# OpenDriveLab/kai0

Measured on AMD Instinct MI355X. Metric: train samples/sec pi0.5 full FT, higher is better.
Workload: dtype bf16; 1 GPU; pi0.5 full fine-tune bf16, batch 32 per MI355X, 3-cam 224x224 (BASELINE.json configs[1]); global_batch=32, seq_len=1018, parallelism=dp1

## Files before the change

kai0_amd/csrc/gemm_bf16.hip:

```cpp
#include "common.h"
#include "../../include/kai0hip.h"
#include <stdlib.h>
#include <algorithm>
#include <atomic>
#include <type_traits>

namespace {

constexpr int BK = 64;

#ifdef KAI0_ABLATE
#define KAI0_ABL(p) ((p).ablate)
#else
#define KAI0_ABL(p) 0
#endif

struct RowMap {
    int32_t rpb;
    int64_t bs, off;
    __device__ __forceinline__ int64_t operator()(int r) const {
        if (rpb == 0) return r;
        const int q = r / rpb;
        return (int64_t)q * bs + (r - q * rpb) + off;
    }
// ... 161 lines not shown
        }
        *reinterpret_cast<f32x4*>(cp) = f32x4{v[0], v[1], v[2], v[3]};
        *reinterpret_cast<f32x4*>(cp + 4) = f32x4{v[4], v[5], v[6], v[7]};
    } else {
        bf16_t* cp = reinterpret_cast<bf16_t*>(cbase) + cz + orow * p.ldc + ccol;
        if (p.nseg > 0) {
            int si = 0;
            if (p.nseg > 1 && ccol >= p.seg_begin[1]) si = 1;
            if (p.nseg > 2 && ccol >= p.seg_begin[2]) si = 2;
            cp = p.seg_dst[si] + orow * p.seg_ld[si] + (ccol - p.seg_begin[si]);
        }
        if (p.accumulate) {
            bf16x8 ov = *reinterpret_cast<const bf16x8*>(cp);
#pragma unroll
            for (int e = 0; e < 8; ++e) v[e] += bf2f(ov[e]);
        }
        bf16x8 ov;
#pragma unroll
        for (int e = 0; e < 8; ++e) ov[e] = f2bf(v[e]);
        store_pre8(cp, ov, p.nt_c);
    }
}

#define N_ALIGNED8(n) (((n) & 7) == 0)

__device__ __forceinline__ void lds_barrier() {
    __builtin_amdgcn_sched_barrier(0);
    asm volatile("s_waitcnt lgkmcnt(0)" ::: "memory");
    __builtin_amdgcn_s_barrier();
    asm volatile("" ::: "memory");
    __builtin_amdgcn_sched_barrier(0);
}

template <bool A_KC, bool B_KC, int WM, int WN, int MT, int NT, bool PP, int NS = 2, int BKT = 64, int SCH = 0>
__global__ __launch_bounds__(WM * WN * 64, (WM * WN * 64) / 256) void gemm_bf16_kernel(const GemmArgs p) {
    static_assert(PP ? (WM == 2 && WN == 4 && MT == 8 && ((SCH == 1 && NS == 2 && BKT == 64) || (SCH == 3 && NS == 4 && BKT == 32)))
                     : (SCH == 0 && NS >= 2 && BKT == 64),
                  "K loops: plain multi-stage (SCH 0, 64 deep), quadrant (SCH 1: 256x256x64, 2 stages), ring (SCH 3: 256x256x32, 4 slots)");
    constexpr int BK = BKT;
    constexpr int NWAVES = WM * WN;
    constexpr int TBM = WM * MT * 16, TBN = WN * NT * 16;
    constexpr int A_TILE = TBM * BK * 2, B_TILE = TBN * BK * 2;
    constexpr int STAGE = A_TILE + B_TILE;
    constexpr int NA = A_TILE / 1024 / NWAVES;
    constexpr int NB = B_TILE / 1024 / NWAVES;
    constexpr int KC_CPR = BK / 8;
// ... 371 lines not shown
    #pragma unroll
                    for (int t = 0; t < AH; ++t) af[t] = load_frag(ta, A_KC, A_ROWB, wm * (MT * 16) + (h * AH + t) * 16, ks);
    #pragma unroll
                    for (int i = 0; i < AH; ++i)
    #pragma unroll
                        for (int j = 0; j < NT; ++j)
                            acc[h * AH + i][j] = __builtin_amdgcn_mfma_f32_16x16x32_bf16(af[i], bfr[j], acc[h * AH + i][j], 0, 0, 0);
                }
            }
            slot_c = slot_c + 1 == NS ? 0 : slot_c + 1;
            slot_p = slot_p + 1 == NS ? 0 : slot_p + 1;
        }
        lds_barrier();
    }

    float* slab = reinterpret_cast<float*>(smem + wave * (AH * 4096));
    const int64_t cz = z1 * p.sC1 + z2 * p.sC2;
    const int64_t rz = z1 * p.sR1 + z2 * p.sR2;
    const int64_t vz = z1 * p.rv_s1 + z2 * p.rv_s2;
    constexpr bool ILM = SCH == 1 && !A_KC, ILN = SCH == 1 && !B_KC;
    const int ccol = ILN ? n0 + ((lane & 7) >> 2) * 128 + wn * 32 + ((lane & 7) & 3) * 8 : n0 + wn * 64 + (lane & 7) * 8;
    auto row_base = [&](int h) { return ILM ? m0 + h * 128 + wm * 64 : m0 + wm * (MT * 16) + h * 64; };
    const bool col_ok = ccol < ((p.N + 7) & ~7);
    const bool fused_fast = p.act >= 2 && p.split_k == 1 && p.bias == nullptr && p.gate == nullptr && p.residual == nullptr &&
                            !p.accumulate && !p.out_f32 && p.nseg == 0 && (p.act == 4 || p.scale == 1.0f) &&
                            (p.act != 3 || p.pre_out != nullptr);
    const bool plain_fast = p.act <= 1 && p.split_k == 1 && (p.bias != nullptr || p.residual != nullptr) && p.gate == nullptr &&
                            !p.accumulate && !p.out_f32 && p.nseg == 0 && (N_ALIGNED8(p.N));
    const bool simple_fast = MT == 8 && p.simple_epi && p.act <= 1 && p.split_k == 1 && p.gate == nullptr && !p.out_f32 && p.scale == 1.0f &&
                             p.cmap.rpb == 0 && (N_ALIGNED8(p.N));
    auto epi_half = [&](auto hc) {
        constexpr int h = decltype(hc)::value;
        if constexpr (((MT == 4 && WM == 2) || (MT == 2 && WM == 4)) && WN == 2 && A_KC && B_KC) if (p.act == 7) {
            const bool rot = n0 < p.rope_n_end;
            const int fi = ((n0 >> 7) & 1) * 64 + (lane & 7) * 8;
            const int rcol = rot ? (n0 >> 8) * 256 + wn * 128 + fi : n0 + wn * 64 + (lane & 7) * 8;
            const int rbase = row_base(h) + (lane >> 3);
            bf16x8 cs[AH * 2], sn[AH * 2];
#pragma unroll
            for (int it = 0; it < AH * 2; ++it) {
                const int64_t tr = (int64_t)min(rbase + it * 8, p.M - 1) * p.rope_half + fi;
                cs[it] = *reinterpret_cast<const bf16x8*>(p.rope_cos + (rot ? tr : 0));
                sn[it] = *reinterpret_cast<const bf16x8*>(p.rope_sin + (rot ? tr : 0));
            }
#pragma unroll
            for (int i = 0; i < AH; ++i)
#pragma unroll
                for (int j = 0; j < 4; ++j)
#pragma unroll
                    for (int r = 0; r < 4; ++r) slab[(i * 16 + 4 * g + r) * 64 + j * 16 + l15] = acc[i][j][r];
            lds_barrier();
            const float* pslab = reinterpret_cast<const float*>(smem + (wave ^ 1) * (AH * 4096));
            int si = 0;
// ... 47 lines not shown
                const float gv[8] = {g0[0], g0[1], g0[2], g0[3], g1[0], g1[1], g1[2], g1[3]};
                const float uv[8] = {u0[0], u0[1], u0[2], u0[3], u1[0], u1[1], u1[2], u1[3]};
                bf16x8 gb, ub, hb;
#pragma unroll
                for (int e = 0; e < 8; e += 2) {
                    const f32x2 gr = rbf2(f32x2{gv[e], gv[e + 1]}), ur = rbf2(f32x2{uv[e], uv[e + 1]});
                    const f32x2 hv = rbf2(gelu_tanh2(gr)) * ur;
                    gb[e] = f2bf(gr[0]);
                    gb[e + 1] = f2bf(gr[1]);
                    ub[e] = f2bf(ur[0]);
                    ub[e + 1] = f2bf(ur[1]);
                    hb[e] = f2bf(hv[0]);
                    hb[e + 1] = f2bf(hv[1]);
                }
                const int64_t o = cz + p.cmap(row) * p.ldc + ocol;
                *reinterpret_cast<bf16x8*>(cb + o) = hb;
                if (p.pre_out != nullptr) store_pre8(p.pre_out + o, gb, p.nt_pre);
                if (p.pre_out2 != nullptr) store_pre8(p.pre_out2 + o, ub, p.nt_pre);
            }
            asm volatile("s_waitcnt lgkmcnt(0)" ::: "memory");
            __builtin_amdgcn_wave_barrier();
            return;
        }
        if constexpr (MT != 2) if (fused_fast) {
            bf16x8 s0[8], s1[8];
            float ds[8];
            const int rbase = row_base(h) + (lane >> 3);
#pragma unroll
            for (int it = 0; it < 8; ++it) {
                const int row = rbase + it * 8;
                s0[it] = bf16x8{};
                s1[it] = bf16x8{};
                ds[it] = 0.f;
                if (row < p.M && col_ok) {
                    const int64_t o = cz + p.cmap(row) * p.ldc + ccol;
                    s0[it] = *reinterpret_cast<const bf16x8*>(p.aux1 + o);
                    if (p.act == 3) s1[it] = *reinterpret_cast<const bf16x8*>(p.aux2 + o);
                    if (p.act == 4) ds[it] = p.rowvec[vz + (int64_t)row * p.rv_ld];
                }
            }
#pragma unroll
            for (int i = 0; i < 4; ++i)
#pragma unroll
                for (int j = 0; j < 4; ++j)
#pragma unroll
                    for (int r = 0; r < 4; ++r) slab[(i * 16 + 4 * g + r) * 64 + j * 16 + l15] = acc[h * 4 + i][j][r];
            asm volatile("s_waitcnt lgkmcnt(0)" ::: "memory");
// ... 110 lines not shown
                        store_pre8(p.pre_out + o, pv, p.nt_pre);
                    }
#pragma unroll
                    for (int e = 0; e < 8; e += 2) {
                        const f32x2 a = gelu_tanh2(f32x2{v[e], v[e + 1]});
                        v[e] = rbf(a[0]);
                        v[e + 1] = rbf(a[1]);
                    }
                }
                if (p.residual != nullptr) {
#pragma unroll
                    for (int e = 0; e < 8; ++e) v[e] = rbf(v[e] + bf2f(rs[it][e]));
                }
                bf16x8 ov;
#pragma unroll
                for (int e = 0; e < 8; ++e) ov[e] = f2bf(v[e]);
                *reinterpret_cast<bf16x8*>(cb + o) = ov;
            }
            asm volatile("s_waitcnt lgkmcnt(0)" ::: "memory");
            __builtin_amdgcn_wave_barrier();
            return;
        }
        if constexpr (MT == 8) if (simple_fast) {
            const bool has_bias = p.bias != nullptr, has_res = p.residual != nullptr, gelu = p.act == 1;
            const int M_ = p.M, nt_pre_ = p.nt_pre, nt_c_ = p.nt_c;
            const bf16_t* res_ = p.residual;
            bf16_t* pre_ = p.pre_out;
            const int64_t ldr_ = p.ldr, ldc_ = p.ldc;
            float bv[8] = {0.f, 0.f, 0.f, 0.f, 0.f, 0.f, 0.f, 0.f};
            if (has_bias && col_ok) {
                if (p.bias_f32) {
                    const f32x4 b0 = *reinterpret_cast<const f32x4*>(reinterpret_cast<const float*>(p.bias) + ccol);
                    const f32x4 b1 = *reinterpret_cast<const f32x4*>(reinterpret_cast<const float*>(p.bias) + ccol + 4);
#pragma unroll
                    for (int e = 0; e < 4; ++e) { bv[e] = b0[e]; bv[4 + e] = b1[e]; }
                } else {
                    const bf16x8 b = *reinterpret_cast<const bf16x8*>(reinterpret_cast<const bf16_t*>(p.bias) + ccol);
#pragma unroll
                    for (int e = 0; e < 8; ++e) bv[e] = bf2f(b[e]);
                }
            }
            bf16_t* cl = reinterpret_cast<bf16_t*>(p.C) + cz + ccol;
            int64_t ldl = p.ldc;
            if (p.nseg > 0) {
                cl = p.seg_dst[0] + (ccol - p.seg_begin[0]);
                ldl = p.seg_ld[0];
                if (p.nseg > 1 && ccol >= p.seg_begin[1]) {
                    cl = p.seg_dst[1] + (ccol - p.seg_begin[1]);
                    ldl = p.seg_ld[1];
                }
                if (p.nseg > 2 && ccol >= p.seg_begin[2]) {
                    cl = p.seg_dst[2] + (ccol - p.seg_begin[2]);
                    ldl = p.seg_ld[2];
                }
            }
            const int rbase = row_base(h) + (lane >> 3);
            auto res_row = [&](int it) -> bf16x8 {
                const int row = rbase + it * 8;
                return (has_res && row < M_ && col_ok) ? *reinterpret_cast<const bf16x8*>(res_ + rz + (int64_t)row * ldr_ + ccol) : bf16x8{};
            };
            const bool accum = p.accumulate != 0;
            auto old_row = [&](int it) -> bf16x8 {
                const int row = rbase + it * 8;
                return (accum && row < M_ && col_ok) ? *reinterpret_cast<const bf16x8*>(cl + (int64_t)row * ldl) : bf16x8{};
            };
            bf16x8 rnext = res_row(0), onext = old_row(0);
#pragma unroll
            for (int i = 0; i < 4; ++i)
#pragma unroll
                for (int j = 0; j < 4; ++j)
#pragma unroll
                    for (int r = 0; r < 4; ++r) slab[(i * 16 + 4 * g + r) * 64 + j * 16 + l15] = acc[h * 4 + i][j][r];
            asm volatile("s_waitcnt lgkmcnt(0)" ::: "memory");
            __builtin_amdgcn_wave_barrier();
#pragma unroll
            for (int it = 0; it < 8; ++it) {
                const int row = rbase + it * 8;
                const float* sp = slab + (it * 8 + (lane >> 3)) * 64 + (lane & 7) * 8;
                const f32x4 v0 = *reinterpret_cast<const f32x4*>(sp);
                const f32x4 v1 = *reinterpret_cast<const f32x4*>(sp + 4);
                const bf16x8 rv = rnext, ov0 = onext;
                if (it + 1 < 8) {
                    rnext = res_row(it + 1);
                    onext = old_row(it + 1);
                }
                if (row >= M_ || !col_ok) continue;
                float v[8] = {v0[0], v0[1], v0[2], v0[3], v1[0], v1[1], v1[2], v1[3]};
                if (has_bias) {
#pragma unroll
                    for (int e = 0; e < 8; ++e) v[e] += bv[e];
                }
#pragma unroll
                for (int e = 0; e < 8; ++e) v[e] = rbf(v[e]);
                if (gelu) {
                    if (pre_ != nullptr) {
                        bf16x8 pv;
#pragma unroll
                        for (int e = 0; e < 8; ++e) pv[e] = f2bf(v[e]);
                        store_pre8(pre_ + cz + (int64_t)row * ldc_ + ccol, pv, nt_pre_);
                    }
#pragma unroll
                    for (int e = 0; e < 8; e += 2) {
                        const f32x2 a = gelu_tanh2(f32x2{v[e], v[e + 1]});
                        v[e] = rbf(a[0]);
                        v[e + 1] = rbf(a[1]);
                    }
                }
                if (has_res) {
#pragma unroll
                    for (int e = 0; e < 8; ++e) v[e] = rbf(v[e] + bf2f(rv[e]));
                }
                if (accum) {
#pragma unroll
                    for (int e = 0; e < 8; ++e) v[e] += bf2f(ov0[e]);
                }
                bf16x8 ov;
#pragma unroll
                for (int e = 0; e < 8; ++e) ov[e] = f2bf(v[e]);
                store_pre8(cl + (int64_t)row * ldl, ov, nt_c_);
            }
            asm volatile("s_waitcnt lgkmcnt(0)" ::: "memory");
            __builtin_amdgcn_wave_barrier();
            return;
        }
#pragma unroll
        for (int i = 0; i < AH; ++i)
#pragma unroll
            for (int j = 0; j < 4; ++j)
#pragma unroll
                for (int r = 0; r < 4; ++r) slab[(i * 16 + 4 * g + r) * 64 + j * 16 + l15] = acc[h * AH + i][j][r];
        asm volatile("s_waitcnt lgkmcnt(0)" ::: "memory");
        __builtin_amdgcn_wave_barrier();
#pragma unroll 1
        for (int it = 0; it < AH * 2; ++it) {
            const int lr = it * 8 + (lane >> 3);
            const int row = row_base(h) + lr;
            if (row >= p.M || !col_ok) continue;
            const float* sp = slab + lr * 64 + (lane & 7) * 8;
            f32x4 v0 = *reinterpret_cast<const f32x4*>(sp);
            f32x4 v1 = *reinterpret_cast<const f32x4*>(sp + 4);
            float v[8] = {v0[0], v0[1], v0[2], v0[3], v1[0], v1[1], v1[2], v1[3]};
            if (p.split_k > 1) {
                float* wp = reinterpret_cast<float*>(p.ws) + ((int64_t)blockIdx.y * p.M + row) * p.N + ccol;
                *reinterpret_cast<f32x4*>(wp) = v0;
                *reinterpret_cast<f32x4*>(wp + 4) = v1;
            } else {
                epilogue8(p, v, row, ccol, cz, rz, vz, p.C, p.out_f32 != 0);
            }
        }
        asm volatile("s_waitcnt lgkmcnt(0)" ::: "memory");
        __builtin_amdgcn_wave_barrier();
    };
    epi_half(std::integral_constant<int, 0>{});
    if constexpr (MT / 4 > 1) epi_half(std::integral_constant<int, 1>{});
    if constexpr (MT / 4 > 2) epi_half(std::integral_constant<int, 2>{});
    static_assert(MT / 4 <= 3, "extend the epilogue parts");
}

constexpr int PS_SLOTS = 1024;
__device__ unsigned int g_ps_ctr[PS_SLOTS][16];

#ifdef KAI0_PS_TRACE
__device__ long long g_ps_trace[256][8];
#define PS_STAMP(i)                                              \
    do {                                                         \
        const long long n_ = __builtin_amdgcn_s_memrealtime();   \
        t_acc[i] += n_ - t_prev;                                 \
        t_prev = n_;                                             \
    } while (0)
#else
#define PS_STAMP(i) do { } while (0)
#endif

__global__ __launch_bounds__(512, 1) void gemm_nt_persistent_kernel(const GemmArgs p, unsigned int* __restrict__ ctr) {
    constexpr int TBM = 256, TBN = 256, A_TILE = TBM * BK * 2, STAGE = 2 * A_TILE, GROUP = 4, MT = 8;
    extern __shared__ __attribute__((aligned(16))) char smem[];
    const int tid = threadIdx.x, lane = tid & 63;
    const int wave = __builtin_amdgcn_readfirstlane(tid >> 6);
// ... 159 lines not shown
            read_a(ta, 1);
            __builtin_amdgcn_sched_barrier(0);
            issue_half(false, 0, t + 2);
            lds_barrier();
            quad(I1{}, I1{});
            lds_barrier();
            read_b(tb, 0);
            __builtin_amdgcn_sched_barrier(0);
            issue_half(true, 1, t + 2);
            asm volatile("s_waitcnt vmcnt(6)" ::: "memory");
            lds_barrier();
            quad(I1{}, I0{});
            lds_barrier();
        }
        asm volatile("s_waitcnt vmcnt(0)" ::: "memory");
        if (grp == 0) lds_barrier();
        lds_barrier();

        PS_STAMP(1);
        const int m0c = m0, n0c = n0;
        int nn = -1;
        unsigned raw = 0;
        if (tid == 0 && nxt >= 0) raw = draw();
        if (nxt >= 0) {
            setup(nxt);
            prologue_issue();
        }
        const int ccol = n0c + wn * 64 + (lane & 7) * 8;
        const bool col_ok = ccol < ((p.N + 7) & ~7);
        const bool fused_fast = p.act >= 2 && p.act <= 5 && p.bias == nullptr && p.gate == nullptr && p.residual == nullptr && !p.accumulate &&
                                !p.out_f32 && p.nseg == 0 && (p.act == 4 || p.scale == 1.0f) && (p.act != 3 || p.pre_out != nullptr);
        const bool simple_fast = p.simple_epi && p.act <= 1 && p.split_k == 1 && p.gate == nullptr && !p.out_f32 && p.scale == 1.0f && p.cmap.rpb == 0 &&
                                 (N_ALIGNED8(p.N));
        auto to_slab = [&](int ti) {
            __builtin_amdgcn_wave_barrier();
#pragma unroll
            for (int j = 0; j < 4; ++j)
#pragma unroll
                for (int r = 0; r < 4; ++r) slab[(4 * g + r) * 64 + j * 16 + l15] = acc[ti][j][r];
            asm volatile("s_waitcnt lgkmcnt(0)" ::: "memory");
            __builtin_amdgcn_wave_barrier();
        };
        if (pair) {
            const int ocol = (n0c >> 1) + wn * 32 + (lane & 3) * 8;
            const bool ocol_ok = ocol < (p.N >> 1);
            bf16_t* cb = reinterpret_cast<bf16_t*>(p.C);
#pragma unroll
            for (int ti = 0; ti < MT; ++ti) {
                to_slab(ti);
                const int row = m0c + wm * 128 + ti * 16 + (lane >> 2);
                const float* sp = slab + (lane >> 2) * 64 + (lane & 3) * 8;
                const f32x4 g0 = *reinterpret_cast<const f32x4*>(sp), g1 = *reinterpret_cast<const f32x4*>(sp + 4);
                const f32x4 u0 = *reinterpret_cast<const f32x4*>(sp + 32), u1 = *reinterpret_cast<const f32x4*>(sp + 36);
                if (row < p.M && ocol_ok) {
                    const float gv[8] = {g0[0], g0[1], g0[2], g0[3], g1[0], g1[1], g1[2], g1[3]};
                    const float uv[8] = {u0[0], u0[1], u0[2], u0[3], u1[0], u1[1], u1[2], u1[3]};
                    bf16x8 gb, ub, hb;
#pragma unroll
                    for (int e = 0; e < 8; e += 2) {
                        const f32x2 gr = rbf2(f32x2{gv[e], gv[e + 1]}), ur = rbf2(f32x2{uv[e], uv[e + 1]});
                        const f32x2 hv = rbf2(gelu_tanh2(gr)) * ur;
                        gb[e] = f2bf(gr[0]); gb[e + 1] = f2bf(gr[1]);
                        ub[e] = f2bf(ur[0]); ub[e + 1] = f2bf(ur[1]);
                        hb[e] = f2bf(hv[0]); hb[e + 1] = f2bf(hv[1]);
                    }
                    const int64_t o = p.cmap(row) * p.ldc + ocol;
                    *reinterpret_cast<bf16x8*>(cb + o) = hb;
                    if (p.pre_out != nullptr) store_pre8(p.pre_out + o, gb, p.nt_pre);
                    if (p.pre_out2 != nullptr) store_pre8(p.pre_out2 + o, ub, p.nt_pre);
                }
            }
        } else if (fused_fast) {
            bf16_t* cb = reinterpret_cast<bf16_t*>(p.C);
#pragma unroll
            for (int h = 0; h < 2; ++h) {
                bf16x8 s0[8], s1[8];
                float ds[8];
                const int rbase = m0c + wm * 128 + h * 64 + (lane >> 3);
#pragma unroll
                for (int it = 0; it < 8; ++it) {
                    const int row = rbase + it * 8;
                    s0[it] = bf16x8{};
                    s1[it] = bf16x8{};
                    ds[it] = 0.f;
                    if (row < p.M && col_ok) {
                        const int64_t o = p.cmap(row) * p.ldc + ccol;
                        s0[it] = *reinterpret_cast<const bf16x8*>(p.aux1 + o);
                        if (p.act == 3) s1[it] = *reinterpret_cast<const bf16x8*>(p.aux2 + o);
                        if (p.act == 4) ds[it] = p.rowvec[(int64_t)row * p.rv_ld];
                    }
                }
#pragma unroll
                for (int i = 0; i < 4; ++i) {
                    to_slab(h * 4 + i);
#pragma unroll
                    for (int it2 = 0; it2 < 2; ++it2) {
                        const int it = 2 * i + it2;
                        const int row = rbase + it * 8;
                        const float* sp = slab + (it2 * 8 + (lane >> 3)) * 64 + (lane & 7) * 8;
                        const f32x4 v0 = *reinterpret_cast<const f32x4*>(sp), v1 = *reinterpret_cast<const f32x4*>(sp + 4);
                        const float v[8] = {v0[0], v0[1], v0[2], v0[3], v1[0], v1[1], v1[2], v1[3]};
                        if (row >= p.M || !col_ok) continue;
                        const int64_t o = p.cmap(row) * p.ldc + ccol;
                        bf16x8 ov;
                        if (p.act == 2) {
                            if (p.pre_out != nullptr) {
                                bf16x8 uv;
#pragma unroll
                                for (int e = 0; e < 8; ++e) uv[e] = f2bf(v[e]);
                                *reinterpret_cast<bf16x8*>(p.pre_out + o) = uv;
                            }
#pragma unroll
                            for (int e = 0; e < 8; e += 2) {
                                const f32x2 r = rbf2(gelu_tanh2(f32x2{bf2f(s0[it][e]), bf2f(s0[it][e + 1])})) * rbf2(f32x2{v[e], v[e + 1]});
                                ov[e] = f2bf(r[0]);
                                ov[e + 1] = f2bf(r[1]);
                            }
                        } else if (p.act == 3) {
                            bf16x8 du;
#pragma unroll
                            for (int e = 0; e < 8; e += 2) {
                                const f32x2 dh = rbf2(f32x2{v[e], v[e + 1]});
                                f32x2 gl, gr;
                                gelu_tanh_both2(f32x2{bf2f(s0[it][e]), bf2f(s0[it][e + 1])}, gl, gr);
                                const f32x2 a = dh * rbf2(gl);
                                const f32x2 b = rbf2(dh * f32x2{bf2f(s1[it][e]), bf2f(s1[it][e + 1])}) * gr;
                                du[e] = f2bf(a[0]); du[e + 1] = f2bf(a[1]);
                                ov[e] = f2bf(b[0]); ov[e + 1] = f2bf(b[1]);
                            }
                            *reinterpret_cast<bf16x8*>(p.pre_out + o) = du;
                        } else if (p.act == 5) {
#pragma unroll
                            for (int e = 0; e < 8; e += 2) {
                                f32x2 gl, gr;
                                gelu_tanh_both2(f32x2{bf2f(s0[it][e]), bf2f(s0[it][e + 1])}, gl, gr);
                                const f32x2 b = rbf2(f32x2{v[e], v[e + 1]}) * gr;
                                ov[e] = f2bf(b[0]); ov[e + 1] = f2bf(b[1]);
                            }
                        } else {
#pragma unroll
                            for (int e = 0; e < 8; ++e) ov[e] = f2bf((bf2f(s0[it][e]) * (v[e] - ds[it])) * p.scale);
                        }
                        *reinterpret_cast<bf16x8*>(cb + o) = ov;
                    }
                }
            }
        } else if (simple_fast) {
            const bool has_bias = p.bias != nullptr, has_res = p.residual != nullptr, gelu = p.act == 1;
            const int M_ = p.M, nt_pre_ = p.nt_pre, nt_c_ = p.nt_c;
            const bf16_t* res_ = p.residual;
            bf16_t* pre_ = p.pre_out;
            const int64_t ldr_ = p.ldr, ldc_ = p.ldc;
            float bv[8] = {0.f, 0.f, 0.f, 0.f, 0.f, 0.f, 0.f, 0.f};
            if (has_bias && col_ok) {
                if (p.bias_f32) {
                    const f32x4 b0 = *reinterpret_cast<const f32x4*>(reinterpret_cast<const float*>(p.bias) + ccol);
                    const f32x4 b1 = *reinterpret_cast<const f32x4*>(reinterpret_cast<const float*>(p.bias) + ccol + 4);
#pragma unroll
                    for (int e = 0; e < 4; ++e) { bv[e] = b0[e]; bv[4 + e] = b1[e]; }
                } else {
                    const bf16x8 b = *reinterpret_cast<const bf16x8*>(reinterpret_cast<const bf16_t*>(p.bias) + ccol);
#pragma unroll
                    for (int e = 0; e < 8; ++e) bv[e] = bf2f(b[e]);
                }
            }
            bf16_t* cl = reinterpret_cast<bf16_t*>(p.C) + ccol;
            int64_t ldl = p.ldc;
            if (p.nseg > 0) {
                cl = p.seg_dst[0] + (ccol - p.seg_begin[0]);
                ldl = p.seg_ld[0];
                if (p.nseg > 1 && ccol >= p.seg_begin[1]) {
                    cl = p.seg_dst[1] + (ccol - p.seg_begin[1]);
                    ldl = p.seg_ld[1];
                }
                if (p.nseg > 2 && ccol >= p.seg_begin[2]) {
                    cl = p.seg_dst[2] + (ccol - p.seg_begin[2]);
                    ldl = p.seg_ld[2];
                }
            }
            const int rbase = m0c + wm * 128 + (lane >> 3);
            auto res_row = [&](int k) -> bf16x8 {
                const int row = rbase + k * 8;
                return (has_res && row < M_ && col_ok) ? *reinterpret_cast<const bf16x8*>(res_ + (int64_t)row * ldr_ + ccol) : bf16x8{};
            };
            const bool accum = p.accumulate != 0;
            auto old_row = [&](int k) -> bf16x8 {
                const int row = rbase + k * 8;
                return (accum && row < M_ && col_ok) ? *reinterpret_cast<const bf16x8*>(cl + (int64_t)row * ldl) : bf16x8{};
            };
            bf16x8 rnext = res_row(0), onext = old_row(0);
#pragma unroll
            for (int ti = 0; ti < MT; ++ti) {
                to_slab(ti);
#pragma unroll
                for (int it2 = 0; it2 < 2; ++it2) {
                    const int k = ti * 2 + it2;
                    const int row = rbase + k * 8;
                    const float* sp = slab + (it2 * 8 + (lane >> 3)) * 64 + (lane & 7) * 8;
                    const f32x4 v0 = *reinterpret_cast<const f32x4*>(sp), v1 = *reinterpret_cast<const f32x4*>(sp + 4);
                    const bf16x8 rv = rnext, ov0 = onext;
                    if (k + 1 < 2 * MT) {
                        rnext = res_row(k + 1);
                        onext = old_row(k + 1);
                    }
                    if (row >= M_ || !col_ok) continue;
                    float v[8] = {v0[0], v0[1], v0[2], v0[3], v1[0], v1[1], v1[2], v1[3]};
                    if (has_bias) {
#pragma unroll
                        for (int e = 0; e < 8; ++e) v[e] += bv[e];
                    }
#pragma unroll
                    for (int e = 0; e < 8; ++e) v[e] = rbf(v[e]);
                    if (gelu) {
                        if (pre_ != nullptr) {
                            bf16x8 pv;
#pragma unroll
                            for (int e = 0; e < 8; ++e) pv[e] = f2bf(v[e]);
                            store_pre8(pre_ + (int64_t)row * ldc_ + ccol, pv, nt_pre_);
                        }
#pragma unroll
                        for (int e = 0; e < 8; e += 2) {
                            const f32x2 a = gelu_tanh2(f32x2{v[e], v[e + 1]});
                            v[e] = rbf(a[0]);
                            v[e + 1] = rbf(a[1]);
                        }
                    }
                    if (has_res) {
#pragma unroll
                        for (int e = 0; e < 8; ++e) v[e] = rbf(v[e] + bf2f(rv[e]));
                    }
                    if (accum) {
#pragma unroll
                        for (int e = 0; e < 8; ++e) v[e] += bf2f(ov0[e]);
                    }
                    bf16x8 ov;
#pragma unroll
                    for (int e = 0; e < 8; ++e) ov[e] = f2bf(v[e]);
                    store_pre8(cl + (int64_t)row * ldl, ov, nt_c_);
                }
            }
        } else {
#pragma unroll
            for (int ti = 0; ti < MT; ++ti) {
                to_slab(ti);
#pragma unroll 1
                for (int it2 = 0; it2 < 2; ++it2) {
                    const int lr = it2 * 8 + (lane >> 3);
                    const int row = m0c + wm * 128 + ti * 16 + lr;
                    if (row >= p.M || !col_ok) continue;
                    const float* sp = slab + lr * 64 + (lane & 7) * 8;
                    const f32x4 v0 = *reinterpret_cast<const f32x4*>(sp), v1 = *reinterpret_cast<const f32x4*>(sp + 4);
                    float v[8] = {v0[0], v0[1], v0[2], v0[3], v1[0], v1[1], v1[2], v1[3]};
                    epilogue8(p, v, row, ccol, cz, rz, vz, p.C, p.out_f32 != 0);
                }
            }
        }
        PS_STAMP(2);
        __builtin_amdgcn_wave_barrier();
        if (tid == 0) mbox[0] = nxt >= 0 ? resolve(raw) : -1;
        asm volatile("s_waitcnt vmcnt(0)" ::: "memory");
        lds_barrier();
        nn = mbox[0];
        cur = nxt;
        nxt = nn;
// ... 374 lines not shown
```

Measured before the change: 68.14 samples/s.

## Prefetch GEMM epilogue operands through a multi-row register ring with specialized fast paths

The fused and simple GEMM epilogues now fetch their auxiliary, residual and accumulate operands EPI_AHEAD row steps ahead into a register ring, instead of one row ahead. The first loads are issued before the accumulator-to-LDS slab write so global memory latency overlaps with that work. Interior tiles get compile-time specialized variants (fixed activation, residual-only or accumulate-only) that drop bounds checks and runtime branches. The cost is more live registers in the epilogue, which may raise register pressure or lower occupancy, plus extra template instantiations.

```diff
diff --git a/kai0_amd/csrc/gemm_bf16.hip b/kai0_amd/csrc/gemm_bf16.hip
--- a/kai0_amd/csrc/gemm_bf16.hip
+++ b/kai0_amd/csrc/gemm_bf16.hip
@@ -207,6 +207,63 @@
     }
 }
 
+template <int ACT>
+__device__ __forceinline__ void fused_row8(const int act_rt, const float scale, const float (&v)[8], const bf16x8 a1, const bf16x8 a2,
+                                           const float dsum, const int64_t o, bf16_t* cb, bf16_t* pre) {
+    const int act = ACT ? ACT : act_rt;
+    bf16x8 ov;
+    if (act == 2) {
+        if (pre != nullptr) {
+            bf16x8 uv;
+#pragma unroll
+            for (int e = 0; e < 8; ++e) uv[e] = f2bf(v[e]);
+            *reinterpret_cast<bf16x8*>(pre + o) = uv;
+        }
+#pragma unroll
+        for (int e = 0; e < 8; e += 2) {
+            const f32x2 r = rbf2(gelu_tanh2(f32x2{bf2f(a1[e]), bf2f(a1[e + 1])})) * rbf2(f32x2{v[e], v[e + 1]});
+            ov[e] = f2bf(r[0]);
+            ov[e + 1] = f2bf(r[1]);
+        }
+    } else if (act == 3) {
+        bf16x8 du;
+#pragma unroll
+        for (int e = 0; e < 8; e += 2) {
+            const f32x2 dh = rbf2(f32x2{v[e], v[e + 1]});
+            f32x2 gl, gr;
+            gelu_tanh_both2(f32x2{bf2f(a1[e]), bf2f(a1[e + 1])}, gl, gr);
+            const f32x2 a = dh * rbf2(gl);
+            const f32x2 b = rbf2(dh * f32x2{bf2f(a2[e]), bf2f(a2[e + 1])}) * gr;
+            du[e] = f2bf(a[0]);
+            du[e + 1] = f2bf(a[1]);
+            ov[e] = f2bf(b[0]);
+            ov[e + 1] = f2bf(b[1]);
+        }
+        *reinterpret_cast<bf16x8*>(pre + o) = du;
+    } else if (act == 5) {
+#pragma unroll
+        for (int e = 0; e < 8; e += 2) {
+            f32x2 gl, gr;
+            gelu_tanh_both2(f32x2{bf2f(a1[e]), bf2f(a1[e + 1])}, gl, gr);
+            const f32x2 b = rbf2(f32x2{v[e], v[e + 1]}) * gr;
+            ov[e] = f2bf(b[0]);
+            ov[e + 1] = f2bf(b[1]);
+        }
+    } else {
+#pragma unroll
+        for (int e = 0; e < 8; ++e) ov[e] = f2bf((bf2f(a1[e]) * (v[e] - dsum)) * scale);
+    }
+    *reinterpret_cast<bf16x8*>(cb + o) = ov;
+}
+
+#ifndef KAI0_EPI_AHEAD
+#define KAI0_EPI_AHEAD 4
+#endif
+constexpr int EPI_AHEAD = KAI0_EPI_AHEAD;
+template <int V>
+using IC = std::integral_constant<int, V>;
+static_assert(EPI_AHEAD >= 1 && EPI_AHEAD <= 8, "the ring holds EPI_AHEAD row steps of operands in registers");
+
 #define N_ALIGNED8(n) (((n) & 7) == 0)
 
 __device__ __forceinline__ void lds_barrier() {
@@ -624,13 +681,20 @@
     const int ccol = ILN ? n0 + ((lane & 7) >> 2) * 128 + wn * 32 + ((lane & 7) & 3) * 8 : n0 + wn * 64 + (lane & 7) * 8;
     auto row_base = [&](int h) { return ILM ? m0 + h * 128 + wm * 64 : m0 + wm * (MT * 16) + h * 64; };
     const bool col_ok = ccol < ((p.N + 7) & ~7);
-    const bool fused_fast = p.act >= 2 && p.split_k == 1 && p.bias == nullptr && p.gate == nullptr && p.residual == nullptr &&
+    const bool fused_fast = p.simple_epi && p.act >= 2 && p.split_k == 1 && p.bias == nullptr && p.gate == nullptr && p.residual == nullptr &&
                             !p.accumulate && !p.out_f32 && p.nseg == 0 && (p.act == 4 || p.scale == 1.0f) &&
                             (p.act != 3 || p.pre_out != nullptr);
     const bool plain_fast = p.act <= 1 && p.split_k == 1 && (p.bias != nullptr || p.residual != nullptr) && p.gate == nullptr &&
                             !p.accumulate && !p.out_f32 && p.nseg == 0 && (N_ALIGNED8(p.N));
     const bool simple_fast = MT == 8 && p.simple_epi && p.act <= 1 && p.split_k == 1 && p.gate == nullptr && !p.out_f32 && p.scale == 1.0f &&
                              p.cmap.rpb == 0 && (N_ALIGNED8(p.N));
+    bf16x8 es0[EPI_AHEAD], es1[EPI_AHEAD];
+    float eds[EPI_AHEAD];
+    float ebv[8];
+    bf16_t* ecl;
+    int64_t eldl;
+    auto step_row = [&](int k) { return row_base(k >> 3) + (k & 7) * 8 + (lane >> 3); };
+    const bool inner = m0 + TBM <= p.M && n0 + TBN <= ((p.N + 7) & ~7);
     auto epi_half = [&](auto hc) {
         constexpr int h = decltype(hc)::value;
         if constexpr (((MT == 4 && WM == 2) || (MT == 2 && WM == 4)) && WN == 2 && A_KC && B_KC) if (p.act == 7) {
@@ -724,7 +788,71 @@
             __builtin_amdgcn_wave_barrier();
             return;
         }
-        if constexpr (MT != 2) if (fused_fast) {
+        if constexpr (MT == 8) if (fused_fast) {
+            const int M_ = p.M, act_ = p.act;
+            auto run_fused = [&](auto actc, auto innerc) {
+                constexpr int ACT = decltype(actc)::value;
+                constexpr bool INNER = decltype(innerc)::value;
+                const float scale_ = p.scale;
+                const RowMap cmap_ = p.cmap;
+                const int64_t ldc_ = p.ldc, rv_ld_ = p.rv_ld;
+                const bf16_t* aux1_ = p.aux1;
+                const bf16_t* aux2_ = p.aux2;
+                const float* rowvec_ = p.rowvec;
+                bf16_t* pre_ = p.pre_out;
+                auto fetch_aux = [&](int k) {
+                    const int row = step_row(k), sl = k % EPI_AHEAD;
+                    es0[sl] = bf16x8{};
+                    es1[sl] = bf16x8{};
+                    eds[sl] = 0.f;
+                    if (INNER || (row < M_ && col_ok)) {
+                        const int64_t o = cz + cmap_(row) * ldc_ + ccol;
+                        es0[sl] = *reinterpret_cast<const bf16x8*>(aux1_ + o);
+                        if (ACT == 3 || (ACT == 0 && act_ == 3)) es1[sl] = *reinterpret_cast<const bf16x8*>(aux2_ + o);
+                        if (ACT == 0 && act_ == 4) eds[sl] = rowvec_[vz + (int64_t)row * rv_ld_];
+                    }
+                };
+                if constexpr (h == 0) {
+#pragma unroll
+                    for (int k = 0; k < EPI_AHEAD; ++k) fetch_aux(k);
+                    __builtin_amdgcn_sched_barrier(0);
+                }
+#pragma unroll
+                for (int i = 0; i < 4; ++i)
+#pragma unroll
+                    for (int j = 0; j < 4; ++j)
+#pragma unroll
+                        for (int r = 0; r < 4; ++r) slab[(i * 16 + 4 * g + r) * 64 + j * 16 + l15] = acc[h * 4 + i][j][r];
+                asm volatile("s_waitcnt lgkmcnt(0)" ::: "memory");
+                __builtin_amdgcn_wave_barrier();
+                bf16_t* cb = reinterpret_cast<bf16_t*>(p.C);
+#pragma unroll
+                for (int it = 0; it < 8; ++it) {
+                    const int k = h * 8 + it;
+                    const int row = step_row(k);
+                    const float* sp = slab + (it * 8 + (lane >> 3)) * 64 + (lane & 7) * 8;
+                    const f32x4 v0 = *reinterpret_cast<const f32x4*>(sp);
+                    const f32x4 v1 = *reinterpret_cast<const f32x4*>(sp + 4);
+                    const float v[8] = {v0[0], v0[1], v0[2], v0[3], v1[0], v1[1], v1[2], v1[3]};
+                    const bf16x8 a1 = es0[k % EPI_AHEAD], a2 = es1[k % EPI_AHEAD];
+                    const float dsum = eds[k % EPI_AHEAD];
+                    if (k + EPI_AHEAD < 16) {
+                        __builtin_amdgcn_sched_barrier(0);
+                        fetch_aux(k + EPI_AHEAD);
+                        __builtin_amdgcn_sched_barrier(0);
+                    }
+                    if (!INNER && (row >= M_ || !col_ok)) continue;
+                    fused_row8<ACT>(act_, scale_, v, a1, a2, dsum, cz + cmap_(row) * ldc_ + ccol, cb, pre_);
+                }
+                asm volatile("s_waitcnt lgkmcnt(0)" ::: "memory");
+                __builtin_amdgcn_wave_barrier();
+            };
+            if (inner && act_ == 3) run_fused(IC<3>{}, std::true_type{});
+            else if (inner && act_ == 5) run_fused(IC<5>{}, std::true_type{});
+            else run_fused(IC<0>{}, std::false_type{});
+            return;
+        }
+        if constexpr (MT == 4) if (fused_fast) {
             bf16x8 s0[8], s1[8];
             float ds[8];
             const int rbase = row_base(h) + (lane >> 3);
@@ -881,105 +1009,121 @@
             return;
         }
         if constexpr (MT == 8) if (simple_fast) {
-            const bool has_bias = p.bias != nullptr, has_res = p.residual != nullptr, gelu = p.act == 1;
+            const bool has_bias = p.bias != nullptr, has_res_ = p.residual != nullptr, gelu_ = p.act == 1, accum_ = p.accumulate != 0;
             const int M_ = p.M, nt_pre_ = p.nt_pre, nt_c_ = p.nt_c;
             const bf16_t* res_ = p.residual;
             bf16_t* pre_ = p.pre_out;
             const int64_t ldr_ = p.ldr, ldc_ = p.ldc;
-            float bv[8] = {0.f, 0.f, 0.f, 0.f, 0.f, 0.f, 0.f, 0.f};
-            if (has_bias && col_ok) {
-                if (p.bias_f32) {
-                    const f32x4 b0 = *reinterpret_cast<const f32x4*>(reinterpret_cast<const float*>(p.bias) + ccol);
-                    const f32x4 b1 = *reinterpret_cast<const f32x4*>(reinterpret_cast<const float*>(p.bias) + ccol + 4);
-#pragma unroll
-                    for (int e = 0; e < 4; ++e) { bv[e] = b0[e]; bv[4 + e] = b1[e]; }
-                } else {
-                    const bf16x8 b = *reinterpret_cast<const bf16x8*>(reinterpret_cast<const bf16_t*>(p.bias) + ccol);
-#pragma unroll
-                    for (int e = 0; e < 8; ++e) bv[e] = bf2f(b[e]);
-                }
-            }
-            bf16_t* cl = reinterpret_cast<bf16_t*>(p.C) + cz + ccol;
-            int64_t ldl = p.ldc;
-            if (p.nseg > 0) {
-                cl = p.seg_dst[0] + (ccol - p.seg_begin[0]);
-                ldl = p.seg_ld[0];
-                if (p.nseg > 1 && ccol >= p.seg_begin[1]) {
-                    cl = p.seg_dst[1] + (ccol - p.seg_begin[1]);
-                    ldl = p.seg_ld[1];
-                }
-                if (p.nseg > 2 && ccol >= p.seg_begin[2]) {
-                    cl = p.seg_dst[2] + (ccol - p.seg_begin[2]);
-                    ldl = p.seg_ld[2];
-                }
-            }
-            const int rbase = row_base(h) + (lane >> 3);
-            auto res_row = [&](int it) -> bf16x8 {
-                const int row = rbase + it * 8;
-                return (has_res && row < M_ && col_ok) ? *reinterpret_cast<const bf16x8*>(res_ + rz + (int64_t)row * ldr_ + ccol) : bf16x8{};
+            if constexpr (h == 0) {
+#pragma unroll
+                for (int e = 0; e < 8; ++e) ebv[e] = 0.f;
+                if (has_bias && col_ok) {
+                    if (p.bias_f32) {
+                        const f32x4 b0 = *reinterpret_cast<const f32x4*>(reinterpret_cast<const float*>(p.bias) + ccol);
+                        const f32x4 b1 = *reinterpret_cast<const f32x4*>(reinterpret_cast<const float*>(p.bias) + ccol + 4);
+#pragma unroll
+                        for (int e = 0; e < 4; ++e) { ebv[e] = b0[e]; ebv[4 + e] = b1[e]; }
+                    } else {
+                        const bf16x8 b = *reinterpret_cast<const bf16x8*>(reinterpret_cast<const bf16_t*>(p.bias) + ccol);
+#pragma unroll
+                        for (int e = 0; e < 8; ++e) ebv[e] = bf2f(b[e]);
+                    }
+                }
+                ecl = reinterpret_cast<bf16_t*>(p.C) + cz + ccol;
+                eldl = p.ldc;
+                if (p.nseg > 0) {
+                    ecl = p.seg_dst[0] + (ccol - p.seg_begin[0]);
+                    eldl = p.seg_ld[0];
+                    if (p.nseg > 1 && ccol >= p.seg_begin[1]) {
+                        ecl = p.seg_dst[1] + (ccol - p.seg_begin[1]);
+                        eldl = p.seg_ld[1];
+                    }
+                    if (p.nseg > 2 && ccol >= p.seg_begin[2]) {
+                        ecl = p.seg_dst[2] + (ccol - p.seg_begin[2]);
+                        eldl = p.seg_ld[2];
+                    }
+                }
+            }
+            auto run_simple = [&](auto modec) {
+                constexpr int MODE = decltype(modec)::value;
+                constexpr bool INNER = MODE != 0;
+                const bool has_res = MODE == 0 ? has_res_ : MODE == 1, accum = MODE == 0 ? accum_ : MODE == 2, gelu = MODE == 0 && gelu_;
+                const bool reads = has_res || accum;
+                bf16_t* cl = ecl;
+                const int64_t ldl = eldl;
+                auto fetch_ro = [&](int k) {
+                    const int row = step_row(k), sl = k % EPI_AHEAD;
+                    const bool ok = INNER || (row < M_ && col_ok);
+                    es0[sl] = (has_res && ok) ? *reinterpret_cast<const bf16x8*>(res_ + rz + (int64_t)row * ldr_ + ccol) : bf16x8{};
+                    es1[sl] = (accum && ok) ? *reinterpret_cast<const bf16x8*>(cl + (int64_t)row * ldl) : bf16x8{};
+                };
+                if constexpr (h == 0) {
+#pragma unroll
+                    for (int k = 0; k < EPI_AHEAD; ++k) fetch_ro(k);
+                    __builtin_amdgcn_sched_barrier(0);
+                }
+#pragma unroll
+                for (int i = 0; i < 4; ++i)
+#pragma unroll
+                    for (int j = 0; j < 4; ++j)
+#pragma unroll
+                        for (int r = 0; r < 4; ++r) slab[(i * 16 + 4 * g + r) * 64 + j * 16 + l15] = acc[h * 4 + i][j][r];
+                asm volatile("s_waitcnt lgkmcnt(0)" ::: "memory");
+                __builtin_amdgcn_wave_barrier();
+#pragma unroll
+                for (int it = 0; it < 8; ++it) {
+                    const int k = h * 8 + it;
+                    const int row = step_row(k);
+                    const float* sp = slab + (it * 8 + (lane >> 3)) * 64 + (lane & 7) * 8;
+                    const f32x4 v0 = *reinterpret_cast<const f32x4*>(sp);
+                    const f32x4 v1 = *reinterpret_cast<const f32x4*>(sp + 4);
+                    const bf16x8 rv = es0[k % EPI_AHEAD], ov0 = es1[k % EPI_AHEAD];
+                    if (k + EPI_AHEAD < 16 && reads) {
+                        __builtin_amdgcn_sched_barrier(0);
+                        fetch_ro(k + EPI_AHEAD);
+                        __builtin_amdgcn_sched_barrier(0);
+                    }
+                    if (!INNER && (row >= M_ || !col_ok)) continue;
+                    float v[8] = {v0[0], v0[1], v0[2], v0[3], v1[0], v1[1], v1[2], v1[3]};
+                    if (has_bias) {
+#pragma unroll
+                        for (int e = 0; e < 8; ++e) v[e] += ebv[e];
+                    }
+#pragma unroll
+                    for (int e = 0; e < 8; ++e) v[e] = rbf(v[e]);
+                    if (gelu) {
+                        if (pre_ != nullptr) {
+                            bf16x8 pv;
+#pragma unroll
+                            for (int e = 0; e < 8; ++e) pv[e] = f2bf(v[e]);
+                            store_pre8(pre_ + cz + (int64_t)row * ldc_ + ccol, pv, nt_pre_);
+                        }
+#pragma unroll
+                        for (int e = 0; e < 8; e += 2) {
+                            const f32x2 a = gelu_tanh2(f32x2{v[e], v[e + 1]});
+                            v[e] = rbf(a[0]);
+                            v[e + 1] = rbf(a[1]);
+                        }
+                    }
+                    if (has_res) {
+#pragma unroll
+                        for (int e = 0; e < 8; ++e) v[e] = rbf(v[e] + bf2f(rv[e]));
+                    }
+                    if (accum) {
+#pragma unroll
+                        for (int e = 0; e < 8; ++e) v[e] += bf2f(ov0[e]);
+                    }
+                    bf16x8 ov;
+#pragma unroll
+                    for (int e = 0; e < 8; ++e) ov[e] = f2bf(v[e]);
+                    store_pre8(cl + (int64_t)row * ldl, ov, nt_c_);
+                }
+                asm volatile("s_waitcnt lgkmcnt(0)" ::: "memory");
+                __builtin_amdgcn_wave_barrier();
             };
-            const bool accum = p.accumulate != 0;
-            auto old_row = [&](int it) -> bf16x8 {
-                const int row = rbase + it * 8;
-                return (accum && row < M_ && col_ok) ? *reinterpret_cast<const bf16x8*>(cl + (int64_t)row * ldl) : bf16x8{};
-            };
-            bf16x8 rnext = res_row(0), onext = old_row(0);
-#pragma unroll
-            for (int i = 0; i < 4; ++i)
-#pragma unroll
-                for (int j = 0; j < 4; ++j)
-#pragma unroll
-                    for (int r = 0; r < 4; ++r) slab[(i * 16 + 4 * g + r) * 64 + j * 16 + l15] = acc[h * 4 + i][j][r];
-            asm volatile("s_waitcnt lgkmcnt(0)" ::: "memory");
-            __builtin_amdgcn_wave_barrier();
-#pragma unroll
-            for (int it = 0; it < 8; ++it) {
-                const int row = rbase + it * 8;
-                const float* sp = slab + (it * 8 + (lane >> 3)) * 64 + (lane & 7) * 8;
-                const f32x4 v0 = *reinterpret_cast<const f32x4*>(sp);
-                const f32x4 v1 = *reinterpret_cast<const f32x4*>(sp + 4);
-                const bf16x8 rv = rnext, ov0 = onext;
-                if (it + 1 < 8) {
-                    rnext = res_row(it + 1);
-                    onext = old_row(it + 1);
-                }
-                if (row >= M_ || !col_ok) continue;
-                float v[8] = {v0[0], v0[1], v0[2], v0[3], v1[0], v1[1], v1[2], v1[3]};
-                if (has_bias) {
-#pragma unroll
-                    for (int e = 0; e < 8; ++e) v[e] += bv[e];
-                }
-#pragma unroll
-                for (int e = 0; e < 8; ++e) v[e] = rbf(v[e]);
-                if (gelu) {
-                    if (pre_ != nullptr) {
-                        bf16x8 pv;
-#pragma unroll
-                        for (int e = 0; e < 8; ++e) pv[e] = f2bf(v[e]);
-                        store_pre8(pre_ + cz + (int64_t)row * ldc_ + ccol, pv, nt_pre_);
-                    }
-#pragma unroll
-                    for (int e = 0; e < 8; e += 2) {
-                        const f32x2 a = gelu_tanh2(f32x2{v[e], v[e + 1]});
-                        v[e] = rbf(a[0]);
-                        v[e + 1] = rbf(a[1]);
-                    }
-                }
-                if (has_res) {
-#pragma unroll
-                    for (int e = 0; e < 8; ++e) v[e] = rbf(v[e] + bf2f(rv[e]));
-                }
-                if (accum) {
-#pragma unroll
-                    for (int e = 0; e < 8; ++e) v[e] += bf2f(ov0[e]);
-                }
-                bf16x8 ov;
-#pragma unroll
-                for (int e = 0; e < 8; ++e) ov[e] = f2bf(v[e]);
-                store_pre8(cl + (int64_t)row * ldl, ov, nt_c_);
-            }
-            asm volatile("s_waitcnt lgkmcnt(0)" ::: "memory");
-            __builtin_amdgcn_wave_barrier();
+            if (inner && !gelu_ && has_res_ && !accum_) run_simple(IC<1>{});
+            else if (inner && !gelu_ && accum_ && !has_res_) run_simple(IC<2>{});
+            else run_simple(IC<0>{});
             return;
         }
 #pragma unroll
@@ -1010,9 +1154,9 @@
         asm volatile("s_waitcnt lgkmcnt(0)" ::: "memory");
         __builtin_amdgcn_wave_barrier();
     };
-    epi_half(std::integral_constant<int, 0>{});
-    if constexpr (MT / 4 > 1) epi_half(std::integral_constant<int, 1>{});
-    if constexpr (MT / 4 > 2) epi_half(std::integral_constant<int, 2>{});
+    epi_half(IC<0>{});
+    if constexpr (MT / 4 > 1) epi_half(IC<1>{});
+    if constexpr (MT / 4 > 2) epi_half(IC<2>{});
     static_assert(MT / 4 <= 3, "extend the epilogue parts");
 }
 
@@ -1218,16 +1362,25 @@
         int nn = -1;
         unsigned raw = 0;
         if (tid == 0 && nxt >= 0) raw = draw();
-        if (nxt >= 0) {
-            setup(nxt);
-            prologue_issue();
-        }
         const int ccol = n0c + wn * 64 + (lane & 7) * 8;
         const bool col_ok = ccol < ((p.N + 7) & ~7);
-        const bool fused_fast = p.act >= 2 && p.act <= 5 && p.bias == nullptr && p.gate == nullptr && p.residual == nullptr && !p.accumulate &&
-                                !p.out_f32 && p.nseg == 0 && (p.act == 4 || p.scale == 1.0f) && (p.act != 3 || p.pre_out != nullptr);
+        const bool fused_fast = p.simple_epi && (p.act == 2 || p.act == 3 || p.act == 5) && p.bias == nullptr && p.gate == nullptr && p.residual == nullptr &&
+                                !p.accumulate && !p.out_f32 && p.nseg == 0 && p.scale == 1.0f && (p.act != 3 || p.pre_out != nullptr);
         const bool simple_fast = p.simple_epi && p.act <= 1 && p.split_k == 1 && p.gate == nullptr && !p.out_f32 && p.scale == 1.0f && p.cmap.rpb == 0 &&
                                  (N_ALIGNED8(p.N));
+        auto hand_over = [&]() {
+            __builtin_amdgcn_sched_barrier(0);
+            setup(max(nxt, 0));
+#pragma unroll
+            for (int x = 0; x < 4; ++x) {
+                ha_off[x] = nxt >= 0 ? ha_off[x] : OOB;
+                hb_off[x] = nxt >= 0 ? hb_off[x] : OOB;
+            }
+            prologue_issue();
+            __builtin_amdgcn_sched_barrier(0);
+        };
+        const bool inner = m0c + TBM <= p.M && n0c + TBN <= ((p.N + 7) & ~7);
+        const int rbase = m0c + wm * 128 + (lane >> 3);
         auto to_slab = [&](int ti) {
             __builtin_amdgcn_wave_barrier();
 #pragma unroll
@@ -1238,6 +1391,7 @@
             __builtin_amdgcn_wave_barrier();
         };
         if (pair) {
+            hand_over();
             const int ocol = (n0c >> 1) + wn * 32 + (lane & 3) * 8;
             const bool ocol_ok = ocol < (p.N >> 1);
             bf16_t* cb = reinterpret_cast<bf16_t*>(p.C);
@@ -1267,82 +1421,56 @@
                 }
             }
         } else if (fused_fast) {
-            bf16_t* cb = reinterpret_cast<bf16_t*>(p.C);
-#pragma unroll
-            for (int h = 0; h < 2; ++h) {
-                bf16x8 s0[8], s1[8];
-                float ds[8];
-                const int rbase = m0c + wm * 128 + h * 64 + (lane >> 3);
-#pragma unroll
-                for (int it = 0; it < 8; ++it) {
-                    const int row = rbase + it * 8;
-                    s0[it] = bf16x8{};
-                    s1[it] = bf16x8{};
-                    ds[it] = 0.f;
-                    if (row < p.M && col_ok) {
-                        const int64_t o = p.cmap(row) * p.ldc + ccol;
-                        s0[it] = *reinterpret_cast<const bf16x8*>(p.aux1 + o);
-                        if (p.act == 3) s1[it] = *reinterpret_cast<const bf16x8*>(p.aux2 + o);
-                        if (p.act == 4) ds[it] = p.rowvec[(int64_t)row * p.rv_ld];
-                    }
-                }
-#pragma unroll
-                for (int i = 0; i < 4; ++i) {
-                    to_slab(h * 4 + i);
+            auto run_fused = [&](auto actc, auto innerc) {
+                constexpr int ACT = decltype(actc)::value;
+                constexpr bool INNER = decltype(innerc)::value;
+                const int M_ = p.M, act_ = p.act;
+                const RowMap cmap_ = p.cmap;
+                const int64_t ldc_ = p.ldc;
+                const bf16_t* aux1_ = p.aux1;
+                const bf16_t* aux2_ = p.aux2;
+                bf16_t* pre_ = p.pre_out;
+                bf16x8 s0[EPI_AHEAD], s1[EPI_AHEAD];
+                auto fetch_aux = [&](int k) {
+                    const int row = rbase + k * 8, sl = k % EPI_AHEAD;
+                    s0[sl] = bf16x8{};
+                    s1[sl] = bf16x8{};
+                    if (INNER || (row < M_ && col_ok)) {
+                        const int64_t o = cmap_(row) * ldc_ + ccol;
+                        s0[sl] = *reinterpret_cast<const bf16x8*>(aux1_ + o);
+                        if (ACT == 3 || (ACT == 0 && act_ == 3)) s1[sl] = *reinterpret_cast<const bf16x8*>(aux2_ + o);
+                    }
+                };
+#pragma unroll
+                for (int k = 0; k < EPI_AHEAD; ++k) fetch_aux(k);
+                hand_over();
+                bf16_t* cb = reinterpret_cast<bf16_t*>(p.C);
+#pragma unroll
+                for (int ti = 0; ti < MT; ++ti) {
+                    to_slab(ti);
 #pragma unroll
                     for (int it2 = 0; it2 < 2; ++it2) {
-                        const int it = 2 * i + it2;
-                        const int row = rbase + it * 8;
+                        const int k = ti * 2 + it2;
+                        const int row = rbase + k * 8;
                         const float* sp = slab + (it2 * 8 + (lane >> 3)) * 64 + (lane & 7) * 8;
                         const f32x4 v0 = *reinterpret_cast<const f32x4*>(sp), v1 = *reinterpret_cast<const f32x4*>(sp + 4);
                         const float v[8] = {v0[0], v0[1], v0[2], v0[3], v1[0], v1[1], v1[2], v1[3]};
-                        if (row >= p.M || !col_ok) continue;
-                        const int64_t o = p.cmap(row) * p.ldc + ccol;
-                        bf16x8 ov;
-                        if (p.act == 2) {
-                            if (p.pre_out != nullptr) {
-                                bf16x8 uv;
-#pragma unroll
-                                for (int e = 0; e < 8; ++e) uv[e] = f2bf(v[e]);
-                                *reinterpret_cast<bf16x8*>(p.pre_out + o) = uv;
-                            }
-#pragma unroll
-                            for (int e = 0; e < 8; e += 2) {
-                                const f32x2 r = rbf2(gelu_tanh2(f32x2{bf2f(s0[it][e]), bf2f(s0[it][e + 1])})) * rbf2(f32x2{v[e], v[e + 1]});
-                                ov[e] = f2bf(r[0]);
-                                ov[e + 1] = f2bf(r[1]);
-                            }
-                        } else if (p.act == 3) {
-                            bf16x8 du;
-#pragma unroll
-                            for (int e = 0; e < 8; e += 2) {
-                                const f32x2 dh = rbf2(f32x2{v[e], v[e + 1]});
-                                f32x2 gl, gr;
-                                gelu_tanh_both2(f32x2{bf2f(s0[it][e]), bf2f(s0[it][e + 1])}, gl, gr);
-                                const f32x2 a = dh * rbf2(gl);
-                                const f32x2 b = rbf2(dh * f32x2{bf2f(s1[it][e]), bf2f(s1[it][e + 1])}) * gr;
-                                du[e] = f2bf(a[0]); du[e + 1] = f2bf(a[1]);
-                                ov[e] = f2bf(b[0]); ov[e + 1] = f2bf(b[1]);
-                            }
-                            *reinterpret_cast<bf16x8*>(p.pre_out + o) = du;
-                        } else if (p.act == 5) {
-#pragma unroll
-                            for (int e = 0; e < 8; e += 2) {
-                                f32x2 gl, gr;
-                                gelu_tanh_both2(f32x2{bf2f(s0[it][e]), bf2f(s0[it][e + 1])}, gl, gr);
-                                const f32x2 b = rbf2(f32x2{v[e], v[e + 1]}) * gr;
-                                ov[e] = f2bf(b[0]); ov[e + 1] = f2bf(b[1]);
-                            }
-                        } else {
-#pragma unroll
-                            for (int e = 0; e < 8; ++e) ov[e] = f2bf((bf2f(s0[it][e]) * (v[e] - ds[it])) * p.scale);
+                        const bf16x8 a1 = s0[k % EPI_AHEAD], a2 = s1[k % EPI_AHEAD];
+                        if (k + EPI_AHEAD < 2 * MT) {
+                            __builtin_amdgcn_sched_barrier(0);
+                            fetch_aux(k + EPI_AHEAD);
+                            __builtin_amdgcn_sched_barrier(0);
                         }
-                        *reinterpret_cast<bf16x8*>(cb + o) = ov;
-                    }
-                }
-            }
+                        if (!INNER && (row >= M_ || !col_ok)) continue;
+                        fused_row8<ACT>(act_, 1.0f, v, a1, a2, 0.f, cmap_(row) * ldc_ + ccol, cb, pre_);
+                    }
+                }
+            };
+            if (inner && p.act == 3) run_fused(IC<3>{}, std::true_type{});
+            else if (inner && p.act == 5) run_fused(IC<5>{}, std::true_type{});
+            else run_fused(IC<0>{}, std::false_type{});
         } else if (simple_fast) {
-            const bool has_bias = p.bias != nullptr, has_res = p.residual != nullptr, gelu = p.act == 1;
+            const bool has_bias = p.bias != nullptr, has_res_ = p.residual != nullptr, gelu_ = p.act == 1, accum_ = p.accumulate != 0;
             const int M_ = p.M, nt_pre_ = p.nt_pre, nt_c_ = p.nt_c;
             const bf16_t* res_ = p.residual;
             bf16_t* pre_ = p.pre_out;
@@ -1374,68 +1502,78 @@
                     ldl = p.seg_ld[2];
                 }
             }
-            const int rbase = m0c + wm * 128 + (lane >> 3);
-            auto res_row = [&](int k) -> bf16x8 {
-                const int row = rbase + k * 8;
-                return (has_res && row < M_ && col_ok) ? *reinterpret_cast<const bf16x8*>(res_ + (int64_t)row * ldr_ + ccol) : bf16x8{};
+            auto run_simple = [&](auto modec) {
+                constexpr int MODE = decltype(modec)::value;
+                constexpr bool INNER = MODE != 0;
+                const bool has_res = MODE == 0 ? has_res_ : MODE == 1, accum = MODE == 0 ? accum_ : MODE == 2, gelu = MODE == 0 && gelu_;
+                const bool reads = has_res || accum;
+                bf16x8 s0[EPI_AHEAD], s1[EPI_AHEAD];
+                auto fetch_ro = [&](int k) {
+                    const int row = rbase + k * 8, sl = k % EPI_AHEAD;
+                    const bool ok = INNER || (row < M_ && col_ok);
+                    s0[sl] = (has_res && ok) ? *reinterpret_cast<const bf16x8*>(res_ + (int64_t)row * ldr_ + ccol) : bf16x8{};
+                    s1[sl] = (accum && ok) ? *reinterpret_cast<const bf16x8*>(cl + (int64_t)row * ldl) : bf16x8{};
+                };
+#pragma unroll
+                for (int k = 0; k < EPI_AHEAD; ++k) fetch_ro(k);
+                hand_over();
+#pragma unroll
+                for (int ti = 0; ti < MT; ++ti) {
+                    to_slab(ti);
+#pragma unroll
+                    for (int it2 = 0; it2 < 2; ++it2) {
+                        const int k = ti * 2 + it2;
+                        const int row = rbase + k * 8;
+                        const float* sp = slab + (it2 * 8 + (lane >> 3)) * 64 + (lane & 7) * 8;
+                        const f32x4 v0 = *reinterpret_cast<const f32x4*>(sp), v1 = *reinterpret_cast<const f32x4*>(sp + 4);
+                        const bf16x8 rv = s0[k % EPI_AHEAD], ov0 = s1[k % EPI_AHEAD];
+                        if (k + EPI_AHEAD < 2 * MT && reads) {
+                            __builtin_amdgcn_sched_barrier(0);
+                            fetch_ro(k + EPI_AHEAD);
+                            __builtin_amdgcn_sched_barrier(0);
+                        }
+                        if (!INNER && (row >= M_ || !col_ok)) continue;
+                        float v[8] = {v0[0], v0[1], v0[2], v0[3], v1[0], v1[1], v1[2], v1[3]};
+                        if (has_bias) {
+#pragma unroll
+                            for (int e = 0; e < 8; ++e) v[e] += bv[e];
+                        }
+#pragma unroll
+                        for (int e = 0; e < 8; ++e) v[e] = rbf(v[e]);
+                        if (gelu) {
+                            if (pre_ != nullptr) {
+                                bf16x8 pv;
+#pragma unroll
+                                for (int e = 0; e < 8; ++e) pv[e] = f2bf(v[e]);
+                                store_pre8(pre_ + (int64_t)row * ldc_ + ccol, pv, nt_pre_);
+                            }
+#pragma unroll
+                            for (int e = 0; e < 8; e += 2) {
+                                const f32x2 a = gelu_tanh2(f32x2{v[e], v[e + 1]});
+                                v[e] = rbf(a[0]);
+                                v[e + 1] = rbf(a[1]);
+                            }
+                        }
+                        if (has_res) {
+#pragma unroll
+                            for (int e = 0; e < 8; ++e) v[e] = rbf(v[e] + bf2f(rv[e]));
+                        }
+                        if (accum) {
+#pragma unroll
+                            for (int e = 0; e < 8; ++e) v[e] += bf2f(ov0[e]);
+                        }
+                        bf16x8 ov;
+#pragma unroll
+                        for (int e = 0; e < 8; ++e) ov[e] = f2bf(v[e]);
+                        store_pre8(cl + (int64_t)row * ldl, ov, nt_c_);
+                    }
+                }
             };
-            const bool accum = p.accumulate != 0;
-            auto old_row = [&](int k) -> bf16x8 {
-                const int row = rbase + k * 8;
-                return (accum && row < M_ && col_ok) ? *reinterpret_cast<const bf16x8*>(cl + (int64_t)row * ldl) : bf16x8{};
-            };
-            bf16x8 rnext = res_row(0), onext = old_row(0);
-#pragma unroll
-            for (int ti = 0; ti < MT; ++ti) {
-                to_slab(ti);
-#pragma unroll
-                for (int it2 = 0; it2 < 2; ++it2) {
-                    const int k = ti * 2 + it2;
-                    const int row = rbase + k * 8;
-                    const float* sp = slab + (it2 * 8 + (lane >> 3)) * 64 + (lane & 7) * 8;
-                    const f32x4 v0 = *reinterpret_cast<const f32x4*>(sp), v1 = *reinterpret_cast<const f32x4*>(sp + 4);
-                    const bf16x8 rv = rnext, ov0 = onext;
-                    if (k + 1 < 2 * MT) {
-                        rnext = res_row(k + 1);
-                        onext = old_row(k + 1);
-                    }
-                    if (row >= M_ || !col_ok) continue;
-                    float v[8] = {v0[0], v0[1], v0[2], v0[3], v1[0], v1[1], v1[2], v1[3]};
-                    if (has_bias) {
-#pragma unroll
-                        for (int e = 0; e < 8; ++e) v[e] += bv[e];
-                    }
-#pragma unroll
-                    for (int e = 0; e < 8; ++e) v[e] = rbf(v[e]);
-                    if (gelu) {
-                        if (pre_ != nullptr) {
-                            bf16x8 pv;
-#pragma unroll
-                            for (int e = 0; e < 8; ++e) pv[e] = f2bf(v[e]);
-                            store_pre8(pre_ + (int64_t)row * ldc_ + ccol, pv, nt_pre_);
-                        }
-#pragma unroll
-                        for (int e = 0; e < 8; e += 2) {
-                            const f32x2 a = gelu_tanh2(f32x2{v[e], v[e + 1]});
-                            v[e] = rbf(a[0]);
-                            v[e + 1] = rbf(a[1]);
-                        }
-                    }
-                    if (has_res) {
-#pragma unroll
-                        for (int e = 0; e < 8; ++e) v[e] = rbf(v[e] + bf2f(rv[e]));
-                    }
-                    if (accum) {
-#pragma unroll
-                        for (int e = 0; e < 8; ++e) v[e] += bf2f(ov0[e]);
-                    }
-                    bf16x8 ov;
-#pragma unroll
-                    for (int e = 0; e < 8; ++e) ov[e] = f2bf(v[e]);
-                    store_pre8(cl + (int64_t)row * ldl, ov, nt_c_);
-                }
-            }
+            if (inner && !gelu_ && has_res_ && !accum_) run_simple(IC<1>{});
+            else if (inner && !gelu_ && accum_ && !has_res_) run_simple(IC<2>{});
+            else run_simple(IC<0>{});
         } else {
+            hand_over();
 #pragma unroll
             for (int ti = 0; ti < MT; ++ti) {
                 to_slab(ti);
```

Measured after the change: 68.78 samples/s, median of 6. No clear change (+0.9%).
